# cloneofsimo/lora

Measured on AMD Instinct MI355X. Metric: train steps/sec SD1.5 rank-4 512^2 (train_lora_dreambooth.py step), higher is better.
Workload: dtype bf16

## Files before the change

include/lora_amd.h:

```cpp
#ifndef LORA_AMD_H
#define LORA_AMD_H

#include <stddef.h>
#include <stdint.h>

#ifdef __cplusplus
extern "C" {
#endif

#define LORA_AMD_ABI_VERSION 7

#define LORA_AMD_OK 0
#define LORA_AMD_EINVAL (-1)
#define LORA_AMD_ERANK (-2)
#define LORA_AMD_ELAUNCH (-3)
#define LORA_AMD_EWORKSPACE (-4)
#define LORA_AMD_EUNSUPPORTED (-5)

#define LORA_AMD_MAX_RANK 64

#define LORA_AMD_F32 0
#define LORA_AMD_F16 1
#define LORA_AMD_BF16 2

// ... 445 lines not shown
                                  int32_t r, int32_t act_dtype, float scale, float dropout_p, uint64_t seed, uint64_t offset,
                                  const uint64_t *offset_dev, void *stream);
int lora_amd_sum_parts(const float *part, int32_t nparts, int64_t stride, float *out, int64_t n, void *stream);


size_t lora_amd_sumsq_workspace(int64_t n);
int lora_amd_sumsq(const float *g, int64_t n, float *out_sumsq, void *workspace,
                   size_t workspace_bytes, void *stream);

typedef struct lora_amd_adamw_group {
  int64_t begin, end;
  float lr;
  float weight_decay;
} lora_amd_adamw_group;

int lora_amd_clip_adamw(float *p, float *g, float *exp_avg, float *exp_avg_sq,
                        int64_t n, const lora_amd_adamw_group *groups_dev,
                        int32_t n_groups, const float *sumsq, float grad_scale,
                        float max_norm, float beta1, float beta2, float eps,
                        int64_t step, int32_t zero_grad, void *stream);

int lora_amd_clip_adamw_dev(float *p, float *g, float *exp_avg, float *exp_avg_sq,
                            int64_t n, const lora_amd_adamw_group *groups_dev,
                            int32_t n_groups, const float *sumsq, float grad_scale,
                            float max_norm, float beta1, float beta2, float eps,
                            const int64_t *step_dev, const float *scaler, int32_t zero_grad, void *stream);
int lora_amd_step_advance(int64_t *step_dev, void *stream);

int lora_amd_loss_scale_update(float *state, const float *sumsq, int64_t *step_dev, float growth_factor,
                               float backoff_factor, int32_t growth_interval, void *stream);

int lora_amd_ti_rows_step(void *table, const void *table_grad, const int64_t *ids_dev, int32_t n_tokens,
                          int32_t hidden, int32_t table_dtype, float *rows, float *exp_avg, float *exp_avg_sq,
                          float lr, float beta1, float beta2, float eps, float weight_decay, float grad_scale,
                          int64_t step, float decay_lambda, float target_norm, void *stream);


size_t lora_amd_groupnorm_workspace(int32_t B, int32_t C, int32_t HW, int32_t groups);
int lora_amd_groupnorm_supported(int32_t B, int32_t C, int32_t HW, int32_t groups);
int lora_amd_groupnorm_fwd(const void *x, const void *gamma, const void *beta, void *y, float *stats,
                           void *workspace, size_t workspace_bytes, int32_t B, int32_t C, int32_t HW,
                           int32_t groups, float eps, int32_t act, int32_t dtype, void *stream);
int lora_amd_groupnorm_bwd(const void *x, const void *gout, const void *gamma, const void *beta,
                           const float *stats, void *dx, void *workspace, size_t workspace_bytes, int32_t B,
                           int32_t C, int32_t HW, int32_t groups, int32_t act, int32_t dtype, void *stream);

size_t lora_amd_groupnorm_nhwc_workspace(int32_t B, int32_t C, int32_t HW, int32_t groups);
int lora_amd_groupnorm_nhwc_fwd(const void *x, const void *gamma, const void *beta, const float *addend, void *y,
                                float *aff, void *workspace, size_t workspace_bytes, int32_t B, int32_t C, int32_t HW,
                                int32_t groups, float eps, int32_t act, int32_t dtype, void *stream);
int lora_amd_groupnorm_nhwc_bwd(const void *x, const void *gout, const void *gamma, const float *aff, void *dx,
                                void *workspace, size_t workspace_bytes, int32_t B, int32_t C, int32_t HW,
                                int32_t groups, int32_t act, int32_t dtype, void *stream);

int lora_amd_layernorm_supported(int32_t K);
int lora_amd_layernorm_fwd(const void *x, const void *gamma, const void *beta, void *y, float *stats, int64_t M,
                           int32_t K, float eps, int32_t dtype, void *stream);
int lora_amd_layernorm_bwd(const void *x, const void *gout, const void *gamma, const float *stats, void *dx,
                           int64_t M, int32_t K, int32_t dtype, void *stream);
int lora_amd_add_layernorm_fwd(const void *x, const void *res, const void *gamma, const void *beta, void *sum_out,
                               void *y, float *stats, int64_t M, int32_t K, float eps, int32_t dtype, void *stream);
int lora_amd_add_layernorm_bwd(const void *x, const void *gout, const void *gsum, const void *gamma,
                               const float *stats, void *dx, int64_t M, int32_t K, int32_t dtype, void *stream);

int lora_amd_geglu_fwd(const void *y, int64_t ldy, void *out, int64_t ldo, int64_t M, int32_t inner, int32_t dtype,
                       void *stream);
int lora_amd_geglu_bwd(const void *y, int64_t ldy, const void *gout, int64_t ldg, void *gy, int64_t ldgy, int64_t M,
                       int32_t inner, int32_t dtype, void *stream);

typedef struct lora_amd_attn_short_plan {
  int32_t run_blocks;
  int32_t slabs;
  int64_t slab_bytes;
  int64_t workspace_bytes;
} lora_amd_attn_short_plan;
int lora_amd_attn_short_bwd_supported(int64_t Sq, int32_t Sk, int32_t D, int32_t dtype, const int64_t *strides_host,
                                      int32_t n_strides);
int lora_amd_attn_short_bwd_plan(int32_t B, int32_t H, int64_t Sq, int32_t Sk, int32_t D,
                                 lora_amd_attn_short_plan *plan_host);
int lora_amd_attn_short_bwd(const void *q, const int64_t *q_strides_host, const void *k,
                            const int64_t *k_strides_host, const void *v, const int64_t *v_strides_host,
                            const void *dout, const int64_t *dout_strides_host, void *dq,
                            const int64_t *dq_strides_host, void *dk, const int64_t *dk_strides_host, void *dv,
                            const int64_t *dv_strides_host, int32_t B, int32_t H, int64_t Sq, int32_t Sk, int32_t D,
                            float scale, int32_t dtype, void *workspace, size_t workspace_bytes, void *stream);

#ifdef __cplusplus
}
#endif
#endif
```

lora_amd/_C.py:

```python
from __future__ import annotations

import ctypes as C
import os
from typing import Dict, Optional, Sequence, Tuple

import torch

_HERE = os.path.dirname(os.path.abspath(__file__))
LIB_PATH = os.path.join(_HERE, "csrc", "liblora_amd.so")

OK = 0
F32, F16, BF16 = 0, 1, 2
FACTOR_RK, FACTOR_KR = 0, 1
ROUND_REFERENCE, ROUND_ONCE, ROUND_DITHER = 0, 1, 2
MAX_RANK = 64
ABI_VERSION = 7

_DT = {torch.float32: F32, torch.float16: F16, torch.bfloat16: BF16}

class HipExtensionMissing(RuntimeError):
    pass


class AttnShortPlan(C.Structure):
# ... 292 lines not shown
    ("lora_amd_linear_ws_heads", cint, (vp, i64, i64, i32, i32, i32, i32, P(WsSite), i32, i32, vp)),
    ("lora_amd_linear_gemm_fwd_heads", cint, (vp, i64, vp, i64, vp, vp, i64, vp, vp, vp, i64, i32, i32, i32, i32,
        f32, f32, i32, i32, i32, i32, i32, i32, vp)),
    ("lora_amd_linear_gemm_fwd_rowscale", cint, (vp, i64, vp, i64, vp, vp, i64, vp, vp, vp, i64, i32, i32, i32, i32,
        f32, vp, i32, i64, i32, vp)),
    ("lora_amd_linear_factors_self_plan", cint, (i64, i32, i32, i32, P(FactorsSelfPlan))),
    ("lora_amd_linear_factors_self_plan_rows", cint, (i64, i32, i32, i32, i32, P(FactorsSelfPlan))),
    ("lora_amd_linear_bwd_factors_self", cint, (vp, i64, vp, i64, vp, vp, vp, vp, i64, i32, i32, i32, i32, f32, i32,
        i32, i32, i32, vp)),
    ("lora_amd_linear_factors_self_ragged_plan", cint, (vp, i32, i32, P(i64))),
    ("lora_amd_linear_bwd_factors_self_ragged", cint, (vp, i32, i64, i32, i32, vp)),
    ("lora_amd_reduce_batched", cint, (vp, i32, i64, vp)),
    ("lora_amd_factors_mfma_plan", cint, (i64, i32, i32, i32, i32, i32, i32, P(FactorsMfmaPlan))),
    ("lora_amd_factor_pack_plan", cint, (P(PackSite), i32, P(i64))),
    ("lora_amd_factor_pack", cint, (vp, i32, i64, i32, vp)),
    ("lora_amd_factors_mfma_ragged_plan", cint, (P(FmSite), i32, i32, i32, P(i64))),
    ("lora_amd_linear_bwd_factors_mfma_ragged", cint, (vp, i32, i64, i32, i32, i32, i32, vp)),
    ("lora_amd_factors_mfma_block_map", cint, (P(FmSite), i32, i64, P(i32))),
    ("lora_amd_linear_bwd_factors_mfma_ragged_mapped", cint, (vp, i32, i64, vp, i32, i32, i32, i32, vp)),
    ("lora_amd_factors_mfma_set_tuning", cint, (i32,)),
    ("lora_amd_conv_plan", cint, (i32, i32, i32, i32, i32, i32, i32, P(ConvPlan))),
    ("lora_amd_conv_down_fwd", cint, (vp, vp, vp, vp, vp, i32, i32, i32, i32, i32, i32, i32, i32, vp)),
    ("lora_amd_conv_up_fwd", cint, (vp, vp, vp, i32, i32, i32, i32, i32, i32, i32, f32, f32, u64, u64, vp, vp)),
    ("lora_amd_conv_up_fwd_rowscale", cint, (vp, vp, vp, i32, i32, i32, i32, i32, i32, i32, f32, vp, i32, i64, f32,
        u64, u64, vp)),
    ("lora_amd_conv_bwd_g", cint, (vp, vp, vp, vp, vp, vp, vp, i32, i32, i32, i32, i32, i32, i32, f32, f32, u64,
        u64, vp, vp)),
    ("lora_amd_conv_bwd_x", cint, (vp, vp, vp, vp, vp, i32, i32, i32, i32, i32, i32, i32, i32, vp)),
    ("lora_amd_conv3_nhwc_plan", cint, (i32, i32, i32, i32, i32, P(Conv3NhwcPlan))),
    ("lora_amd_conv3_nhwc_pack", cint, (vp, i32, i32, i32, vp, vp, vp)),
    ("lora_amd_conv3_nhwc_down_fwd", cint, (vp, vp, vp, vp, i32, i32, i32, i32, i32, i32, vp)),
    ("lora_amd_conv3_nhwc_bwd_dx", cint, (vp, vp, vp, i32, i32, i32, i32, i32, i32, vp)),
    ("lora_amd_conv3_nhwc_bwd_down", cint, (vp, vp, vp, i32, i32, i32, i32, i32, i32, vp)),
    ("lora_amd_conv3_nhwc_pack_plan", cint, (P(Conv3PackSite), i32, P(i64))),
    ("lora_amd_conv3_nhwc_pack_batched", cint, (vp, i32, i64, i32, vp)),
    ("lora_amd_conv3_nhwc_fwd_fused", cint, (vp, vp, vp, vp, vp, vp, vp, i32, i32, i32, i32, i32, i32, i32, f32,
        f32, u64, u64, vp, vp)),
    ("lora_amd_sum_parts", cint, (vp, i32, i64, vp, i64, vp)),
    ("lora_amd_sumsq_workspace", sz, (i64,)),
    ("lora_amd_sumsq", cint, (vp, i64, vp, vp, sz, vp)),
    ("lora_amd_clip_adamw", cint, (vp, vp, vp, vp, i64, vp, i32, vp, f32, f32, f32, f32, f32, i64, i32, vp)),
    ("lora_amd_clip_adamw_dev", cint, (vp, vp, vp, vp, i64, vp, i32, vp, f32, f32, f32, f32, f32, vp, vp, i32, vp)),
    ("lora_amd_step_advance", cint, (vp, vp)),
    ("lora_amd_loss_scale_update", cint, (vp, vp, vp, f32, f32, i32, vp)),
    ("lora_amd_ti_rows_step", cint, (vp, vp, vp, i32, i32, i32, vp, vp, vp, f32, f32, f32, f32, f32, f32, i64, f32,
        f32, vp)),
    ("lora_amd_groupnorm_workspace", sz, (i32, i32, i32, i32)),
    ("lora_amd_groupnorm_supported", cint, (i32, i32, i32, i32)),
    ("lora_amd_groupnorm_fwd", cint, (vp, vp, vp, vp, vp, vp, sz, i32, i32, i32, i32, f32, i32, i32, vp)),
    ("lora_amd_groupnorm_bwd", cint, (vp, vp, vp, vp, vp, vp, vp, sz, i32, i32, i32, i32, i32, i32, vp)),
    ("lora_amd_groupnorm_nhwc_workspace", sz, (i32, i32, i32, i32)),
    ("lora_amd_groupnorm_nhwc_fwd", cint, (vp, vp, vp, vp, vp, vp, vp, sz, i32, i32, i32, i32, f32, i32, i32, vp)),
    ("lora_amd_groupnorm_nhwc_bwd", cint, (vp, vp, vp, vp, vp, vp, sz, i32, i32, i32, i32, i32, i32, vp)),
    ("lora_amd_layernorm_supported", cint, (i32,)),
    ("lora_amd_layernorm_fwd", cint, (vp, vp, vp, vp, vp, i64, i32, f32, i32, vp)),
    ("lora_amd_layernorm_bwd", cint, (vp, vp, vp, vp, vp, i64, i32, i32, vp)),
    ("lora_amd_add_layernorm_fwd", cint, (vp, vp, vp, vp, vp, vp, vp, i64, i32, f32, i32, vp)),
    ("lora_amd_add_layernorm_bwd", cint, (vp, vp, vp, vp, vp, vp, i64, i32, i32, vp)),
    ("lora_amd_geglu_fwd", cint, (vp, i64, vp, i64, i64, i32, i32, vp)),
    ("lora_amd_geglu_bwd", cint, (vp, i64, vp, i64, vp, i64, i64, i32, i32, vp)),
    ("lora_amd_attn_short_bwd_supported", cint, (i64, i32, i32, i32, vp, i32)),
    ("lora_amd_attn_short_bwd_plan", cint, (i32, i32, i64, i32, i32, P(AttnShortPlan))),
    ("lora_amd_attn_short_bwd", cint, (vp, vp, vp, vp, vp, vp, vp, vp, vp, vp, vp, vp, vp, vp, i32, i32, i64, i32,
        i32, f32, i32, vp, sz, vp)),
)
SYMBOLS = tuple(name for name, _, _ in FUNCTIONS)


_lib: Optional[C.CDLL] = None
_load_error: Optional[str] = None


def _declare(lib: C.CDLL) -> None:
    for name, restype, argtypes in FUNCTIONS:
        fn = getattr(lib, name)
        fn.restype, fn.argtypes = restype, list(argtypes)


def load() -> Optional[C.CDLL]:
    global _lib, _load_error
    if _lib is not None or _load_error is not None:
        return _lib
    if not os.path.exists(LIB_PATH):
        _load_error = f"{LIB_PATH} not built (run `python -c 'import __graft_entry__ as g; g.build()'`)"
        return None
    try:
        lib = C.CDLL(LIB_PATH)
        _declare(lib)
        if lib.lora_amd_abi_version() != ABI_VERSION:
            raise OSError(f"ABI version {lib.lora_amd_abi_version()} != {ABI_VERSION} (rebuild: make -C lora_amd/csrc)")
        _lib = lib
    except OSError as e:
        _load_error = f"cannot load {LIB_PATH}: {e}"
    return _lib


def available() -> bool:
    return load() is not None


def require() -> C.CDLL:
    lib = load()
    if lib is None:
        raise HipExtensionMissing(
            "lora_amd: the HIP extension is required for device tensors and is not loadable: " + str(_load_error))
    return lib
# ... 1519 lines not shown
    elif out.dtype != y.dtype or tuple(out.shape) != shape or not out.is_contiguous():
        raise ValueError(f"geglu_fwd: out must be a contiguous {y.dtype} {list(shape)} tensor")
    _check(require().lora_amd_geglu_fwd(y2.data_ptr(), y2.stride(0), out.data_ptr(), inner, y2.shape[0], inner,
                                        dtype_code(y.dtype), _stream()), "lora_amd_geglu_fwd")
    return out


def geglu_bwd(y: torch.Tensor, gout: torch.Tensor) -> torch.Tensor:
    _dev_check(y, gout)
    y2, g2 = _as2d(y.reshape(-1, y.shape[-1])), _as2d(gout.reshape(-1, gout.shape[-1]))
    inner = y2.shape[1] // 2
    gy = torch.empty(y.shape, dtype=y.dtype, device=y.device)
    _check(require().lora_amd_geglu_bwd(y2.data_ptr(), y2.stride(0), g2.data_ptr(), g2.stride(0), gy.data_ptr(),
                                        2 * inner, y2.shape[0], inner, dtype_code(y.dtype), _stream()),
           "lora_amd_geglu_bwd")
    return gy


def layernorm_supported(K: int) -> bool:
    return bool(require().lora_amd_layernorm_supported(K))


def layernorm_fwd(x: torch.Tensor, gamma: torch.Tensor, beta: torch.Tensor, eps: float, *,
                  out: Optional[torch.Tensor] = None, stats: Optional[torch.Tensor] = None) -> Tuple[torch.Tensor, torch.Tensor]:
    _dev_check(x, gamma, beta, out, stats)
    K = x.shape[-1]
    M = x.numel() // K
    if out is None:
        y = torch.empty_like(x)
    elif out.dtype != x.dtype or out.shape != x.shape or not out.is_contiguous():
        raise ValueError("layernorm_fwd: out must be a contiguous tensor of x's shape and dtype")
    else:
        y = out
    if stats is None:
        stats = torch.empty(M, 2, dtype=torch.float32, device=x.device)
    elif stats.dtype != torch.float32 or tuple(stats.shape) != (M, 2) or not stats.is_contiguous():
        raise ValueError(f"layernorm_fwd: stats must be a contiguous f32 [{M}, 2] tensor")
    _check(require().lora_amd_layernorm_fwd(x.data_ptr(), gamma.data_ptr(), beta.data_ptr(), y.data_ptr(),
                                            stats.data_ptr(), M, K, eps, dtype_code(x.dtype), _stream()),
           "lora_amd_layernorm_fwd")
    return y, stats


def layernorm_bwd(x: torch.Tensor, gout: torch.Tensor, gamma: torch.Tensor, stats: torch.Tensor) -> torch.Tensor:
    _dev_check(x, gout, gamma, stats)
    K = x.shape[-1]
    dx = torch.empty_like(x)
    _check(require().lora_amd_layernorm_bwd(x.data_ptr(), gout.data_ptr(), gamma.data_ptr(), stats.data_ptr(),
                                            dx.data_ptr(), x.numel() // K, K, dtype_code(x.dtype), _stream()),
           "lora_amd_layernorm_bwd")
    return dx


_gn_nhwc_ws_cache: Dict[Tuple[int, int, int, int], int] = {}


def groupnorm_nhwc_workspace(B: int, C_: int, HW: int, groups: int) -> int:
    key = (B, C_, HW, groups)
    n = _gn_nhwc_ws_cache.get(key)
    if n is None:
        n = _gn_nhwc_ws_cache[key] = int(require().lora_amd_groupnorm_nhwc_workspace(B, C_, HW, groups))
    return n


def groupnorm_nhwc_fwd(x: torch.Tensor, gamma: torch.Tensor, beta: torch.Tensor, groups: int, eps: float,
                       act: bool, addend: Optional[torch.Tensor] = None) -> Tuple[torch.Tensor, torch.Tensor]:
    _dev_check(x, gamma, beta, addend)
    if addend is not None and (addend.dtype != torch.float32 or not addend.is_contiguous()
                               or tuple(addend.shape) != (x.shape[0], x.shape[1])):
        raise ValueError("groupnorm_nhwc_fwd: addend must be a contiguous float32 [B, C] tensor")
    B, C_ = x.shape[0], x.shape[1]
    HW = x.numel() // (B * C_)
    nbytes = groupnorm_nhwc_workspace(B, C_, HW, groups)
    if nbytes == 0:
        raise ValueError(f"lora_amd_groupnorm_nhwc: geometry {tuple(x.shape)} / {groups} groups not supported")
    y = torch.empty_like(x)
    aff = torch.empty(B, 4, C_, dtype=torch.float32, device=x.device)
    ws = torch.empty(nbytes // 4, dtype=torch.float32, device=x.device)
    _check(require().lora_amd_groupnorm_nhwc_fwd(x.data_ptr(), gamma.data_ptr(), beta.data_ptr(), _ptr(addend),
                                                 y.data_ptr(), aff.data_ptr(), ws.data_ptr(), nbytes, B, C_, HW, groups, eps,
                                                 1 if act else 0, dtype_code(x.dtype), _stream()),
           "lora_amd_groupnorm_nhwc_fwd")
    return y, aff


def groupnorm_nhwc_bwd(x: torch.Tensor, gout: torch.Tensor, gamma: torch.Tensor, aff: torch.Tensor, groups: int,
                       act: bool) -> torch.Tensor:
    _dev_check(x, gout, gamma, aff)
    B, C_ = x.shape[0], x.shape[1]
    HW = x.numel() // (B * C_)
    nbytes = groupnorm_nhwc_workspace(B, C_, HW, groups)
    dx = torch.empty_like(x)
    ws = torch.empty(nbytes // 4, dtype=torch.float32, device=x.device)
    _check(require().lora_amd_groupnorm_nhwc_bwd(x.data_ptr(), gout.data_ptr(), gamma.data_ptr(), aff.data_ptr(),
                                                 dx.data_ptr(), ws.data_ptr(), nbytes, B, C_, HW, groups,
                                                 1 if act else 0, dtype_code(x.dtype), _stream()),
           "lora_amd_groupnorm_nhwc_bwd")
    return dx


def add_layernorm_fwd(x: torch.Tensor, res: torch.Tensor, gamma: torch.Tensor, beta: torch.Tensor,
                      eps: float) -> Tuple[torch.Tensor, torch.Tensor, torch.Tensor]:
    _dev_check(x, res, gamma, beta)
    K = x.shape[-1]
    M = x.numel() // K
    s, y = torch.empty_like(x), torch.empty_like(x)
# ... 81 lines not shown
```

lora_amd/csrc/hostops.hip:

```cpp
#include <algorithm>

#include "common.hpp"

namespace lora_amd {

constexpr int kHT = 256;
constexpr int kHU = 4;
constexpr int kHMaxSlices = 256;

__device__ inline float fast_rcp(float v) { return __builtin_amdgcn_rcpf(v); }
__device__ inline float sigmoidf(float z) { return fast_rcp(1.f + __expf(-z)); }
__device__ inline float silu_grad(float z) {
  const float s = sigmoidf(z);
  return s * (1.f + z * (1.f - s));
}
__device__ inline float erf_as(float x) {
  const float ax = fabsf(x);
  const float t = fast_rcp(1.f + 0.3275911f * ax);
  float p = 1.061405429f;
  p = fmaf(p, t, -1.453152027f);
  p = fmaf(p, t, 1.421413741f);
  p = fmaf(p, t, -0.284496736f);
  p = fmaf(p, t, 0.254829592f);
  const float e = 1.f - p * t * __expf(-ax * ax);
// ... 752 lines not shown
      }
      LORA_AMD_LOADS_ISSUED();
#pragma unroll
      for (int u = 0; u < kNU; ++u) {
        const int pp = p + u * nslots;
        if (pp < k.np) {
          float v[8], go[8], t[8], xh[8];
          unpack8_sel<E>(xr[u], true, v);
          unpack8_sel<E>(gr[u], true, go);
          gn_nhwc_terms<E, ACT>(v, go, ga, be, mean, rstd, gam, t, xh);
          if (APPLY) {
            float o[8];
#pragma unroll
            for (int e = 0; e < 8; ++e) o[e] = rstd[e] * (t[e] - c1[e] - xh[e] * c2[e]);
            store8<E>(dx + k.base + (int64_t)pp * C, o);
          } else {
#pragma unroll
            for (int e = 0; e < 8; ++e) {
              s1[e] += t[e];
              s2[e] = fmaf(t[e], xh[e], s2[e]);
            }
          }
        }
      }
    }
  }
  if (!APPLY) {
    nhwc_slot_reduce(s1, s2, k, cw, nslots, s_red);
    if (k.active && k.slot == 0) {
      float *o = part + ((int64_t)(k.b * S + k.s) * 2) * C + (int64_t)k.col * 8;
      st8f(o, s1);
      st8f(o + C, s2);
    }
  }
}

__global__ __launch_bounds__(kHT) void gn_nhwc_bwd_finalize_kernel(const float *__restrict__ part,
                                                                   float *__restrict__ cvec, int C, int HW, int G,
                                                                   int S) {
  __shared__ float s_red[4][2];
  const int b = blockIdx.x / G, g = blockIdx.x - b * G, cpg = C / G;
  float s1 = 0.f, s2 = 0.f;
  for (int i = threadIdx.x; i < S * cpg; i += kHT) {
    const int s = i / cpg, c = g * cpg + (i - s * cpg);
    const float *pp = part + ((int64_t)(b * S + s) * 2) * C + c;
    s1 += pp[0];
    s2 += pp[C];
  }
  block_sum2(s1, s2, s_red);
  const float inv_n = 1.f / ((float)HW * (float)cpg);
  for (int cc = threadIdx.x; cc < cpg; cc += kHT) {
    cvec[(int64_t)b * 2 * C + g * cpg + cc] = s1 * inv_n;
    cvec[(int64_t)b * 2 * C + C + g * cpg + cc] = s2 * inv_n;
  }
}

static inline bool aligned_for(const void *p, int dt) { return ((uintptr_t)p % (dt == LORA_AMD_F32 ? 32 : 16)) == 0; }

}

using namespace lora_amd;

extern "C" size_t lora_amd_groupnorm_workspace(int32_t B, int32_t C, int32_t HW, int32_t groups) {
  const GnGeo q = gn_geo(B, C, HW, groups);
  return q.ok ? (size_t)B * groups * q.S * 2 * sizeof(float) : 0;
}

extern "C" int lora_amd_groupnorm_supported(int32_t B, int32_t C, int32_t HW, int32_t groups) {
  return gn_geo(B, C, HW, groups).ok ? 1 : 0;
}

#define GN_CHECKS(name)                                                                                              \
  const GnGeo q = gn_geo(B, C, HW, groups);                                                                          \
  LORA_AMD_CHECK(q.ok, LORA_AMD_EINVAL, name ": geometry B=%d C=%d HW=%d groups=%d not supported", B, C, HW, groups); \
  LORA_AMD_CHECK(dtype_ok(dtype), LORA_AMD_EINVAL, name ": bad dtype %d", dtype);                                    \
  LORA_AMD_CHECK(workspace_bytes >= lora_amd_groupnorm_workspace(B, C, HW, groups), LORA_AMD_EWORKSPACE,             \
                 name ": workspace %zu < %zu bytes", workspace_bytes, lora_amd_groupnorm_workspace(B, C, HW, groups)); \
  const dim3 grid((unsigned)((int64_t)B * groups * q.S)), block(kHT);                                                \
  hipStream_t st = (hipStream_t)stream;                                                                              \
  float *part = reinterpret_cast<float *>(workspace)

extern "C" int lora_amd_groupnorm_fwd(const void *x, const void *gamma, const void *beta, void *y, float *stats,
                                      void *workspace, size_t workspace_bytes, int32_t B, int32_t C, int32_t HW,
                                      int32_t groups, float eps, int32_t act, int32_t dtype, void *stream) {
  GN_CHECKS("groupnorm_fwd");
  LORA_AMD_CHECK(x && gamma && beta && y && stats && workspace, LORA_AMD_EINVAL, "groupnorm_fwd: null pointer");
  LORA_AMD_CHECK(aligned_for(x, dtype) && aligned_for(y, dtype), LORA_AMD_EINVAL, "groupnorm_fwd: unaligned tensor");
  by_dtype(dtype, [&](auto e) {
    using E = decltype(e);
    using S = typename E::storage;
    hipLaunchKernelGGL((gn_stats_kernel<E>), grid, block, 0, st, (const S *)x, part, groups, q.cpg, HW, q.chunks,
                       q.per_block, q.S);
    by_bool(act != 0, [&](auto a) {
      hipLaunchKernelGGL((gn_apply_kernel<E, decltype(a)::value>), grid, block, 0, st, (const S *)x, (const S *)gamma,
                         (const S *)beta, (S *)y, part, stats, groups, q.cpg, HW, q.chunks, q.per_block, q.S, eps);
    });
  });
  return check_launch("lora_amd_groupnorm_fwd");
}

extern "C" int lora_amd_groupnorm_bwd(const void *x, const void *gout, const void *gamma, const void *beta,
                                      const float *stats, void *dx, void *workspace, size_t workspace_bytes,
                                      int32_t B, int32_t C, int32_t HW, int32_t groups, int32_t act, int32_t dtype,
                                      void *stream) {
  GN_CHECKS("groupnorm_bwd");
  LORA_AMD_CHECK(x && gout && gamma && beta && stats && dx && workspace, LORA_AMD_EINVAL,
// ... 89 lines not shown
  const bool add = res != nullptr;
  by_dtype(dtype, [&](auto e) {
    by_bool(add, [&](auto a) {
      using S = typename decltype(e)::storage;
      hipLaunchKernelGGL((ln_fwd_kernel<decltype(e), decltype(a)::value>), grid, block, 0, st, (const S *)x, (const S *)res,
                         (const S *)gamma, (const S *)beta, (S *)sum_out, (S *)y, stats, M, c8, logL, eps);
    });
  });
  return check_launch("lora_amd_layernorm_fwd");
}

extern "C" int lora_amd_layernorm_bwd(const void *x, const void *gout, const void *gamma, const float *stats,
                                      void *dx, int64_t M, int32_t K, int32_t dtype, void *stream) {
  return lora_amd_add_layernorm_bwd(x, gout, nullptr, gamma, stats, dx, M, K, dtype, stream);
}

extern "C" int lora_amd_add_layernorm_bwd(const void *x, const void *gout, const void *gsum, const void *gamma,
                                          const float *stats, void *dx, int64_t M, int32_t K, int32_t dtype,
                                          void *stream) {
  LN_CHECKS("layernorm_bwd");
  LORA_AMD_CHECK(x && gout && gamma && stats && dx, LORA_AMD_EINVAL, "layernorm_bwd: null pointer");
  LORA_AMD_CHECK(aligned_for(x, dtype) && aligned_for(gout, dtype) && aligned_for(dx, dtype) && aligned_for(gamma, dtype) &&
                     aligned_for(gsum, dtype),
                 LORA_AMD_EINVAL, "layernorm_bwd: unaligned tensor");
  by_dtype(dtype, [&](auto e) {
    by_bool(gsum != nullptr, [&](auto a) {
      using S = typename decltype(e)::storage;
      hipLaunchKernelGGL((ln_bwd_kernel<decltype(e), decltype(a)::value>), grid, block, 0, st, (const S *)x, (const S *)gout,
                         (const S *)gsum, (const S *)gamma, stats, (S *)dx, M, c8, logL);
    });
  });
  return check_launch("lora_amd_layernorm_bwd");
}

static size_t gn_nhwc_part_floats(const GnNhwcGeo &q, int B, int C) { return (size_t)B * q.S * 2 * C; }

extern "C" size_t lora_amd_groupnorm_nhwc_workspace(int32_t B, int32_t C, int32_t HW, int32_t groups) {
  const GnNhwcGeo q = gn_nhwc_geo(B, C, HW, groups);
  return q.ok ? (gn_nhwc_part_floats(q, B, C) + (size_t)B * 2 * C) * sizeof(float) : 0;
}

#define GN_NHWC_CHECKS(name)                                                                                          \
  const GnNhwcGeo q = gn_nhwc_geo(B, C, HW, groups);                                                                  \
  LORA_AMD_CHECK(q.ok, LORA_AMD_EINVAL, name ": geometry B=%d C=%d HW=%d groups=%d not supported", B, C, HW, groups); \
  LORA_AMD_CHECK(dtype_ok(dtype), LORA_AMD_EINVAL, name ": bad dtype %d", dtype);                                     \
  LORA_AMD_CHECK(workspace_bytes >= lora_amd_groupnorm_nhwc_workspace(B, C, HW, groups), LORA_AMD_EWORKSPACE,         \
                 name ": workspace %zu bytes too small", workspace_bytes);                                            \
  const dim3 grid((unsigned)((int64_t)B * q.S * q.tiles)), gridg((unsigned)(B * groups)), block(kHT);                 \
  hipStream_t st = (hipStream_t)stream;                                                                               \
  float *part = reinterpret_cast<float *>(workspace);                                                                 \
  float *cvec = part + gn_nhwc_part_floats(q, B, C);                                                                  \
  (void)cvec

extern "C" int lora_amd_groupnorm_nhwc_fwd(const void *x, const void *gamma, const void *beta, const float *addend,
                                           void *y, float *aff, void *workspace, size_t workspace_bytes, int32_t B, int32_t C, int32_t HW,
                                           int32_t groups, float eps, int32_t act, int32_t dtype, void *stream) {
  GN_NHWC_CHECKS("groupnorm_nhwc_fwd");
  LORA_AMD_CHECK(x && gamma && beta && y && aff && workspace, LORA_AMD_EINVAL, "groupnorm_nhwc_fwd: null pointer");
  LORA_AMD_CHECK(aligned_for(x, dtype) && aligned_for(y, dtype) && ((uintptr_t)aff % 32) == 0, LORA_AMD_EINVAL,
                 "groupnorm_nhwc_fwd: unaligned tensor");
  by_dtype(dtype, [&](auto e) {
    using E = decltype(e);
    using S = typename E::storage;
    hipLaunchKernelGGL((gn_nhwc_stats_kernel<E>), grid, block, 0, st, (const S *)x, part, C, HW, q.cw, q.tiles,
                       q.nslots, q.px, q.S);
    hipLaunchKernelGGL((gn_nhwc_finalize_kernel<E>), gridg, block, 0, st, part, (const S *)gamma, (const S *)beta,
                       addend, aff, C, HW, groups, q.px, q.S, eps);
    by_bool(act != 0, [&](auto a) {
      hipLaunchKernelGGL((gn_nhwc_apply_kernel<E, decltype(a)::value>), grid, block, 0, st, (const S *)x, aff, (S *)y, C, HW,
                         q.cw, q.tiles, q.nslots, q.px, q.S);
    });
  });
  return check_launch("lora_amd_groupnorm_nhwc_fwd");
}

extern "C" int lora_amd_groupnorm_nhwc_bwd(const void *x, const void *gout, const void *gamma, const float *aff,
                                           void *dx, void *workspace, size_t workspace_bytes, int32_t B, int32_t C,
                                           int32_t HW, int32_t groups, int32_t act, int32_t dtype, void *stream) {
  GN_NHWC_CHECKS("groupnorm_nhwc_bwd");
  LORA_AMD_CHECK(x && gout && gamma && aff && dx && workspace, LORA_AMD_EINVAL, "groupnorm_nhwc_bwd: null pointer");
  LORA_AMD_CHECK(aligned_for(x, dtype) && aligned_for(gout, dtype) && aligned_for(dx, dtype) &&
                     aligned_for(gamma, dtype) && ((uintptr_t)aff % 32) == 0,
                 LORA_AMD_EINVAL, "groupnorm_nhwc_bwd: unaligned tensor");
  by_dtype(dtype, [&](auto e) {
    by_bool(act != 0, [&](auto a) {
      using E = decltype(e);
      using S = typename E::storage;
      constexpr bool A = decltype(a)::value;
      hipLaunchKernelGGL((gn_nhwc_bwd_kernel<E, A, false>), grid, block, 0, st, (const S *)x, (const S *)gout,
                         (const S *)gamma, aff, part, (const float *)nullptr, (S *)nullptr, C, HW, q.cw, q.tiles,
                         q.nslots, q.px, q.S);
      hipLaunchKernelGGL(gn_nhwc_bwd_finalize_kernel, gridg, block, 0, st, part, cvec, C, HW, groups, q.S);
      hipLaunchKernelGGL((gn_nhwc_bwd_kernel<E, A, true>), grid, block, 0, st, (const S *)x, (const S *)gout,
                         (const S *)gamma, aff, (float *)nullptr, cvec, (S *)dx, C, HW, q.cw, q.tiles, q.nslots,
                         q.px, q.S);
    });
  });
  return check_launch("lora_amd_groupnorm_nhwc_bwd");
}
```

lora_amd/ops.py:

```python
from __future__ import annotations

import os

from typing import NamedTuple, Optional

import torch
import torch.nn.functional as F

from . import _C

def next_dropout_stream(device) -> tuple:
    seed = int(torch.initial_seed()) & 0xFFFFFFFFFFFFFFFF
    pool = _POOL.get("buf")
    if pool is not None and pool.device == torch.device(device):
        i = _POOL["next"]
        if i >= pool.numel():
            pool = _POOL["buf"] = torch.empty(_POOL_SIZE, dtype=torch.int64, device=device).random_(0, 1 << 62)
            i = 0
        _POOL["next"] = i + 1
        return seed, pool[i:i + 1]
    off = torch.empty(1, dtype=torch.int64, device=device).random_(0, 1 << 62)
    return seed, off


# ... 385 lines not shown
            _log("bwd", "g+lib+x", M, K, N, r)
            gt_part, up_part, down_part = bufs()
            _C.linear_bwd_g(g2, t, up_c, gt_part, up_part, s, p, seed, off)
            dx2 = (g2 @ weight) if need_x else None
            if dx2 is not None and not _C._rows_ok(dx2):
                dx2 = dx2.contiguous()
            _C.linear_bwd_x(x2, dx2, gt_part, plan.nct_g, down_c, sel, down_part)
        if need_x:
            dx = dx2.view(x_shape)
        if not deferred:
            d_down, d_up = _finish(sink, site, bufs(), down, up)
    else:
        gt = None
        _log("bwd", "primitives", M, K, N, r)
        if need_x or need_down:
            gt = rowdot_any(g2, up_c, _C.FACTOR_KR, s, sel, True, p, seed, off)
        if need_up:
            if sink is not None:
                colreduce_any(g2, t, _C.FACTOR_KR, s, out=sink.up_grad, beta=1.0, p=p, seed=seed, off=off)
            else:
                d_up = colreduce_any(g2, t, _C.FACTOR_KR, s, p=p, seed=seed, off=off).to(up.dtype)
        if need_down:
            if sink is not None:
                colreduce_any(x2, gt, _C.FACTOR_RK, 1.0, out=sink.down_grad, beta=1.0)
            else:
                d_down = colreduce_any(x2, gt, _C.FACTOR_RK, 1.0).to(down.dtype)
        if need_x:
            dx2 = g2 @ weight
            rank_update_any_(dx2, gt, down_c, _C.FACTOR_RK, 1.0)
            dx = dx2.view(x_shape)
    dw = g2.t() @ x2 if need_w else None
    db = g2.sum(0) if (has_bias and need_b) else None
    return dx, dw, db, d_down, d_up


def _linear_backward_unpacked(ctx, g2, drop=(0.0, 0, 0)):
    x2, weight, down, up, t = ctx.saved_tensors[:5]
    x_log = unpack_heads(x2, ctx.in_heads) if ctx.in_heads else x2
    g_log = unpack_heads(g2, ctx.out_heads) if ctx.out_heads else g2
    dx, dw, db, d_down, d_up = _linear_backward(
        (x_log, weight, down, up, t, None), ctx.needs_input_grad[:5], g_log, ctx.scale, drop, ctx.sink,
        _C.fused_ok(x_log, weight.shape[0], down.shape[0]), ctx.has_bias, x_log.shape)
    if dx is not None:
        if ctx.in_heads:
            dx = pack_heads(dx, ctx.in_heads)
        dx = dx.view(*ctx.x_shape[:-1], dx.shape[-1])
    return dx, dw, db, d_down, d_up


CONCAT_GROUPS = True
CONV3_FUSED = True
MASTER_MERGE = True
ATTN_SHORT_BWD = True


def apply_ab_overrides(spec: str, namespace: dict) -> dict:
    allowed = ("ATTN_SHORT_BWD", "CONCAT_GROUPS", "CONV3_FUSED", "MASTER_MERGE", "WS_HEADS", "WS_DROPOUT", "WS_DROPOUT_WIDE",
               "WS_DROPOUT_WIDE_BWD")
    done = {}
    for item in filter(None, (s.strip() for s in spec.split(","))):
        name, _, val = item.partition("=")
        if name not in allowed:
            raise ValueError(f"LORA_AMD_AB: unknown constant {name!r} (one of {', '.join(allowed)})")
        namespace[name] = done[name] = val.strip() not in ("0", "", "false", "False")
    return done


apply_ab_overrides(os.environ.get("LORA_AMD_AB", ""), globals())

MERGE_ROUNDING = _C.ROUND_ONCE if os.environ.get("LORA_AMD_MERGE_ROUNDING", "dither") == "once" else _C.ROUND_DITHER


def master_site(w: torch.Tensor, dt: torch.dtype) -> bool:
    return MASTER_MERGE and w.dtype == torch.float32 and dt in (torch.bfloat16, torch.float16) and not w.requires_grad


def _gemm_range():
    if PATH_LOG is not None:
        return torch.profiler.record_function("lora_amd::merged_gemm")
    import contextlib

    return contextlib.nullcontext()


class MergedWeights:

    def __init__(self, state=None):
        self.entries = {}
        self._plans = None
        self.refreshes = 0
        self._state = state
        self._fresh_at = None
        self.defer_factors = state is not None
        self._owed = []
        self._tables = {}
        self._packs = {}
        self._pack_tables = {}
        self._graph_keep = []
        self.groups = {}
        self._keys = {}

    def lookup(self, module, w, b, dt, in_heads, out_heads, need_dx: bool = True):
        e = self._entry(module, w, b, dt, in_heads, out_heads)
        if need_dx and e["w_eff_t"] is None and (e["step"] or (in_heads is None and w.shape[0] % 32 == 0)):
            self._add_transposed(e)
        return e["w_eff"], e["b_eff"], e["w_eff_t"]

    def _refresh_if_stale(self) -> None:
        if (self._state is not None and self._fresh_at != self._state.step_count
                and not torch.cuda.is_current_stream_capturing()):
            self.refresh()

    def _entry(self, module, w, b, dt, in_heads, out_heads, out=None):
        self._refresh_if_stale()
        key = (id(module), in_heads, out_heads, dt)
        e = self.entries.get(key)
        if e is not None and (e["ptrs"] != (module.lora_up.weight.data_ptr(), module.lora_down.weight.data_ptr(),
                                            w.data_ptr()) or e["scale"] != float(module.scale)):
            if e.get("group") is not None:
                self.groups.pop(e["group"], None)
            e = None
# ... 1077 lines not shown
```

Baseline: 36.75.

## Add single-launch NHWC groupnorm forward/backward kernels for small spatial sizes

Adds one-kernel NHWC groupnorm forward and backward paths for HW up to 256. Each block keeps its pixel tile in registers and reduces group statistics in LDS with compensated sums, replacing the stats/finalize/apply sequence of three launches and the workspace round-trips. The path is on by default and can be switched off with an A/B override. In exchange, small-HW layers run with fewer blocks per launch and higher register pressure from the per-thread tiles.

New measurement: 36.97 (median of 4 runs). About the same (+0.6%).

```diff
diff --git a/include/lora_amd.h b/include/lora_amd.h
--- a/include/lora_amd.h
+++ b/include/lora_amd.h
@@ -521,6 +521,7 @@
 int lora_amd_groupnorm_nhwc_bwd(const void *x, const void *gout, const void *gamma, const float *aff, void *dx,
                                 void *workspace, size_t workspace_bytes, int32_t B, int32_t C, int32_t HW,
                                 int32_t groups, int32_t act, int32_t dtype, void *stream);
+int lora_amd_groupnorm_nhwc_set_tuning(int32_t one_launch);
 
 int lora_amd_layernorm_supported(int32_t K);
 int lora_amd_layernorm_fwd(const void *x, const void *gamma, const void *beta, void *y, float *stats, int64_t M,
diff --git a/lora_amd/_C.py b/lora_amd/_C.py
--- a/lora_amd/_C.py
+++ b/lora_amd/_C.py
@@ -368,6 +368,7 @@
     ("lora_amd_groupnorm_nhwc_workspace", sz, (i32, i32, i32, i32)),
     ("lora_amd_groupnorm_nhwc_fwd", cint, (vp, vp, vp, vp, vp, vp, vp, sz, i32, i32, i32, i32, f32, i32, i32, vp)),
     ("lora_amd_groupnorm_nhwc_bwd", cint, (vp, vp, vp, vp, vp, vp, sz, i32, i32, i32, i32, i32, i32, vp)),
+    ("lora_amd_groupnorm_nhwc_set_tuning", cint, (i32,)),
     ("lora_amd_layernorm_supported", cint, (i32,)),
     ("lora_amd_layernorm_fwd", cint, (vp, vp, vp, vp, vp, i64, i32, f32, i32, vp)),
     ("lora_amd_layernorm_bwd", cint, (vp, vp, vp, vp, vp, i64, i32, i32, vp)),
@@ -1993,6 +1994,10 @@
     return dx
 
 
+def groupnorm_nhwc_set_tuning(one_launch: int = -1) -> int:
+    return int(require().lora_amd_groupnorm_nhwc_set_tuning(int(one_launch)))
+
+
 _gn_nhwc_ws_cache: Dict[Tuple[int, int, int, int], int] = {}
 
 
diff --git a/lora_amd/csrc/hostops.hip b/lora_amd/csrc/hostops.hip
--- a/lora_amd/csrc/hostops.hip
+++ b/lora_amd/csrc/hostops.hip
@@ -828,6 +828,284 @@
   for (int cc = threadIdx.x; cc < cpg; cc += kHT) {
     cvec[(int64_t)b * 2 * C + g * cpg + cc] = s1 * inv_n;
     cvec[(int64_t)b * 2 * C + C + g * cpg + cc] = s2 * inv_n;
+  }
+}
+
+constexpr int kGnOneMaxHW = 256;
+constexpr int kGnOneMaxChunks = 32;
+
+struct GnOneGeo {
+  int cpg, nchunk, nblk, nslots, R;
+  bool ok;
+};
+static GnOneGeo gn_one_geo(int B, int C, int HW, int G, int dtype) {
+  GnOneGeo o{};
+  if (!(B > 0 && C > 0 && HW > 0 && G > 0 && C % G == 0 && C % 8 == 0)) return o;
+  o.cpg = C / G;
+  int cb = o.cpg;
+  while (cb % 8) cb += o.cpg;
+  o.nchunk = cb / 8;
+  o.nblk = C / cb;
+  if (HW > kGnOneMaxHW || o.nchunk > kGnOneMaxChunks) return o;
+  o.nslots = std::min(kHT / o.nchunk, HW);
+  o.R = (HW + o.nslots - 1) / o.nslots;
+  o.ok = o.R <= (dtype == LORA_AMD_F32 ? 8 : 16);
+  return o;
+}
+
+struct GnOneBlock {
+  int b, slot, cl, c;
+  bool active;
+  int64_t base;
+};
+__device__ inline GnOneBlock gn_one_block(int C, int HW, int nchunk, int nblk, int nslots) {
+  GnOneBlock k;
+  k.b = blockIdx.x / nblk;
+  const int blk = blockIdx.x - k.b * nblk;
+  k.slot = threadIdx.x / nchunk;
+  k.cl = (threadIdx.x - k.slot * nchunk) * 8;
+  k.active = k.slot < nslots;
+  k.c = blk * nchunk * 8 + k.cl;
+  k.base = (int64_t)k.b * HW * C + k.c;
+  return k;
+}
+
+struct GnOneLds {
+  float red[2 * kHT * 8];
+  float part[2][kHT];
+  float grp[2][kGnOneMaxChunks * 8];
+  float sh[kGnOneMaxChunks * 8];
+  float ad[kGnOneMaxChunks * 8];
+};
+
+__device__ inline void two_add(float &hi, float &lo, float v) {
+  const float t = hi + v, bb = t - hi;
+  lo += (hi - (t - bb)) + (v - bb);
+  hi = t;
+}
+__device__ inline void wave_two_sum(float &hi, float &lo) {
+#pragma unroll
+  for (int off = 32; off > 0; off >>= 1) {
+    const float oh = __shfl_xor(hi, off, 64), ol = __shfl_xor(lo, off, 64);
+    two_add(hi, lo, oh);
+    lo += ol;
+  }
+  const float t = hi + lo;
+  lo = (hi - t) + lo;
+  hi = t;
+}
+
+template <bool MEAN>
+__device__ inline void gn_one_group_avg(float (&a0)[8], float (&a1)[8], const GnOneBlock &k, int nchunk, int nslots, int cpg,
+                                        float denom, float inv_hw, GnOneLds &s) {
+  const int cb = nchunk * 8;
+  const int P = max(1, min(kHT / cb, nslots));
+  __syncthreads();
+  if (k.active) {
+    st8f(s.red + (size_t)threadIdx.x * 8, a0);
+    if (!MEAN) st8f(s.red + (size_t)(kHT + threadIdx.x) * 8, a1);
+  }
+  __syncthreads();
+  if ((int)threadIdx.x < P * cb) {
+    const int cls = threadIdx.x / cb, j = threadIdx.x - cls * cb;
+    float v0 = 0.f, v1 = 0.f;
+#pragma unroll 4
+    for (int sl = cls; sl < nslots; sl += P) {
+      v0 += s.red[sl * cb + j];
+      if (!MEAN) v1 += s.red[kHT * 8 + sl * cb + j];
+    }
+    s.part[0][threadIdx.x] = v0;
+    if (!MEAN) s.part[1][threadIdx.x] = v1;
+  }
+  __syncthreads();
+  const int wave = threadIdx.x >> 6, lane = threadIdx.x & 63;
+  for (int g = wave; g < cb / cpg; g += kHT / 64) {
+    float h0 = 0.f, l0 = 0.f, h1 = 0.f, l1 = 0.f;
+    for (int i = lane; i < P * cpg; i += 64) {
+      const int cls = i / cpg, j = g * cpg + (i - cls * cpg);
+      if (MEAN) {
+        two_add(h0, l0, s.part[0][cls * cb + j] * inv_hw);
+        if (cls == 0) {
+          two_add(h0, l0, s.sh[j]);
+          two_add(h0, l0, s.ad[j]);
+        }
+      } else {
+        two_add(h0, l0, s.part[0][cls * cb + j]);
+        two_add(h1, l1, s.part[1][cls * cb + j]);
+      }
+    }
+    wave_two_sum(h0, l0);
+    if (!MEAN) wave_two_sum(h1, l1);
+    if (lane == 0) {
+      const float q = h0 / denom;
+      s.grp[0][g] = q;
+      s.grp[1][g] = MEAN ? (fmaf(-q, denom, h0) + l0) / denom : h1 / denom;
+    }
+  }
+  __syncthreads();
+#pragma unroll
+  for (int e = 0; e < 8; ++e) {
+    const int g = (k.cl + e) / cpg;
+    a0[e] = s.grp[0][g];
+    a1[e] = s.grp[1][g];
+  }
+}
+
+template <class E, bool ACT, int R>
+__global__ __launch_bounds__(kHT) void gn_nhwc_one_fwd_kernel(const typename E::storage *__restrict__ x,
+                                                              const typename E::storage *__restrict__ gamma,
+                                                              const typename E::storage *__restrict__ beta,
+                                                              const float *__restrict__ addend,
+                                                              typename E::storage *__restrict__ y,
+                                                              float *__restrict__ aff, int C, int HW, int cpg, int nchunk,
+                                                              int nblk, int nslots, float eps) {
+  __shared__ __attribute__((aligned(16))) GnOneLds s;
+  const GnOneBlock k = gn_one_block(C, HW, nchunk, nblk, nslots);
+  Raw8<E> raw[R];
+#pragma unroll
+  for (int u = 0; u < R; ++u) {
+    const int pp = k.slot + u * nslots;
+    raw[u] = load8_raw<E>(x + k.base + (int64_t)(k.active && pp < HW ? pp : 0) * C);
+  }
+  const Raw8<E> shr = load8_raw<E>(x + k.base);
+  const Raw8<E> gr = load8_raw<E>(gamma + k.c), br = load8_raw<E>(beta + k.c);
+  float add[8];
+#pragma unroll
+  for (int e = 0; e < 8; ++e) add[e] = 0.f;
+  if (addend != nullptr) ld8f(addend + (int64_t)k.b * C + k.c, add);
+  LORA_AMD_LOADS_ISSUED();
+  float sh[8], a0[8], a1[8];
+  unpack8_sel<E>(shr, true, sh);
+#pragma unroll
+  for (int e = 0; e < 8; ++e) a0[e] = a1[e] = 0.f;
+#pragma unroll
+  for (int u = 0; u < R; ++u) {
+    float v[8];
+    unpack8_sel<E>(raw[u], true, v);
+    if (k.active && k.slot + u * nslots < HW) {
+#pragma unroll
+      for (int e = 0; e < 8; ++e) a0[e] += v[e] - sh[e];
+    }
+  }
+  if (k.slot == 0) {
+#pragma unroll
+    for (int e = 0; e < 8; ++e) {
+      s.sh[k.cl + e] = sh[e];
+      s.ad[k.cl + e] = add[e];
+    }
+  }
+  gn_one_group_avg<true>(a0, a1, k, nchunk, nslots, cpg, (float)cpg, 1.f / (float)HW, s);
+  float mc[8], ml[8];
+#pragma unroll
+  for (int e = 0; e < 8; ++e) {
+    float hi = a0[e], lo = a1[e];
+    two_add(hi, lo, -add[e]);
+    mc[e] = hi + lo;
+    ml[e] = (hi - mc[e]) + lo;
+    a0[e] = a1[e] = 0.f;
+  }
+#pragma unroll
+  for (int u = 0; u < R; ++u) {
+    float v[8];
+    unpack8_sel<E>(raw[u], true, v);
+    if (k.active && k.slot + u * nslots < HW) {
+#pragma unroll
+      for (int e = 0; e < 8; ++e) {
+        const float d = (v[e] - mc[e]) - ml[e];
+        a0[e] = fmaf(d, d, a0[e]);
+      }
+    }
+  }
+  gn_one_group_avg<false>(a0, a1, k, nchunk, nslots, cpg, (float)HW * (float)cpg, 0.f, s);
+  float gam[8], bet[8], ga[8], be[8], rstd[8];
+  unpack8_sel<E>(gr, true, gam);
+  unpack8_sel<E>(br, true, bet);
+#pragma unroll
+  for (int e = 0; e < 8; ++e) {
+    rstd[e] = rsqrtf(a0[e] + eps);
+    ga[e] = gam[e] * rstd[e];
+    be[e] = fmaf(-mc[e], ga[e], fmaf(-ml[e], ga[e], bet[e]));
+  }
+  if (!k.active) return;
+  if (k.slot == 0) {
+    float *o = aff + (int64_t)k.b * 4 * C + k.c;
+    st8f(o, ga);
+    st8f(o + C, be);
+    st8f(o + 2 * C, mc);
+    st8f(o + 3 * C, rstd);
+  }
+#pragma unroll
+  for (int u = 0; u < R; ++u) {
+    const int pp = k.slot + u * nslots;
+    if (pp < HW) {
+      float v[8], o[8];
+      unpack8_sel<E>(raw[u], true, v);
+#pragma unroll
+      for (int e = 0; e < 8; ++e) {
+        const float z = fmaf((v[e] - mc[e]) - ml[e], ga[e], bet[e]);
+        o[e] = ACT ? z * sigmoidf(z) : z;
+      }
+      store8<E>(y + k.base + (int64_t)pp * C, o);
+    }
+  }
+}
+
+template <class E, bool ACT, int R>
+__global__ __launch_bounds__(kHT) void gn_nhwc_one_bwd_kernel(const typename E::storage *__restrict__ x,
+                                                              const typename E::storage *__restrict__ gout,
+                                                              const typename E::storage *__restrict__ gamma,
+                                                              const float *__restrict__ aff,
+                                                              typename E::storage *__restrict__ dx, int C, int HW, int cpg,
+                                                              int nchunk, int nblk, int nslots) {
+  __shared__ __attribute__((aligned(16))) GnOneLds s;
+  const GnOneBlock k = gn_one_block(C, HW, nchunk, nblk, nslots);
+  Raw8<E> xr[R], gr[R];
+#pragma unroll
+  for (int u = 0; u < R; ++u) {
+    const int pp = k.slot + u * nslots;
+    const int64_t off = k.base + (int64_t)(k.active && pp < HW ? pp : 0) * C;
+    xr[u] = load8_raw<E>(x + off);
+    gr[u] = load8_raw<E>(gout + off);
+  }
+  float ga[8], be[8], mean[8], rstd[8], gam[8], s1[8], s2[8];
+  const float *ab = aff + (int64_t)k.b * 4 * C + k.c;
+  ld8f(ab, ga);
+  ld8f(ab + C, be);
+  ld8f(ab + 2 * C, mean);
+  ld8f(ab + 3 * C, rstd);
+  const Raw8<E> gmr = load8_raw<E>(gamma + k.c);
+  LORA_AMD_LOADS_ISSUED();
+  unpack8_sel<E>(gmr, true, gam);
+#pragma unroll
+  for (int e = 0; e < 8; ++e) s1[e] = s2[e] = 0.f;
+#pragma unroll
+  for (int u = 0; u < R; ++u) {
+    float v[8], go[8], t[8], xh[8];
+    unpack8_sel<E>(xr[u], true, v);
+    unpack8_sel<E>(gr[u], true, go);
+    gn_nhwc_terms<E, ACT>(v, go, ga, be, mean, rstd, gam, t, xh);
+    if (k.active && k.slot + u * nslots < HW) {
+#pragma unroll
+      for (int e = 0; e < 8; ++e) {
+        s1[e] += t[e];
+        s2[e] = fmaf(t[e], xh[e], s2[e]);
+      }
+    }
+  }
+  gn_one_group_avg<false>(s1, s2, k, nchunk, nslots, cpg, (float)HW * (float)cpg, 0.f, s);
+  if (!k.active) return;
+#pragma unroll
+  for (int u = 0; u < R; ++u) {
+    const int pp = k.slot + u * nslots;
+    if (pp < HW) {
+      float v[8], go[8], t[8], xh[8], o[8];
+      unpack8_sel<E>(xr[u], true, v);
+      unpack8_sel<E>(gr[u], true, go);
+      gn_nhwc_terms<E, ACT>(v, go, ga, be, mean, rstd, gam, t, xh);
+#pragma unroll
+      for (int e = 0; e < 8; ++e) o[e] = rstd[e] * (t[e] - s1[e] - xh[e] * s2[e]);
+      store8<E>(dx + k.base + (int64_t)pp * C, o);
+    }
   }
 }
 
@@ -1023,6 +1301,28 @@
   float *cvec = part + gn_nhwc_part_floats(q, B, C);                                                                  \
   (void)cvec
 
+static int g_gn_one_launch = 1;
+static unsigned g_gn_one_count = 0;
+
+extern "C" int lora_amd_groupnorm_nhwc_set_tuning(int32_t one_launch) {
+  if (one_launch == -2) return (int)(g_gn_one_count & 0x7fffffffu);
+  const int prev = g_gn_one_launch;
+  if (one_launch == 0 || one_launch == 1) g_gn_one_launch = one_launch;
+  return prev;
+}
+
+template <class E, class F>
+static void gn_one_by_tile(int R, F &&f) {
+  if (R <= 2) return f(int_c<2>);
+  if (R <= 4) return f(int_c<4>);
+  if constexpr (std::is_same<E, f32_t>::value) {
+    return f(int_c<8>);
+  } else {
+    if (R <= 8) return f(int_c<8>);
+    return f(int_c<16>);
+  }
+}
+
 extern "C" int lora_amd_groupnorm_nhwc_fwd(const void *x, const void *gamma, const void *beta, const float *addend,
                                            void *y, float *aff, void *workspace, size_t workspace_bytes, int32_t B, int32_t C, int32_t HW,
                                            int32_t groups, float eps, int32_t act, int32_t dtype, void *stream) {
@@ -1030,9 +1330,23 @@
   LORA_AMD_CHECK(x && gamma && beta && y && aff && workspace, LORA_AMD_EINVAL, "groupnorm_nhwc_fwd: null pointer");
   LORA_AMD_CHECK(aligned_for(x, dtype) && aligned_for(y, dtype) && ((uintptr_t)aff % 32) == 0, LORA_AMD_EINVAL,
                  "groupnorm_nhwc_fwd: unaligned tensor");
+  const GnOneGeo o = gn_one_geo(B, C, HW, groups, dtype);
+  const bool one = g_gn_one_launch != 0 && o.ok && aligned_for(gamma, dtype) && aligned_for(beta, dtype) &&
+                   ((uintptr_t)addend % 16) == 0;
   by_dtype(dtype, [&](auto e) {
     using E = decltype(e);
     using S = typename E::storage;
+    if (one) {
+      ++g_gn_one_count;
+      by_bool(act != 0, [&](auto a) {
+        gn_one_by_tile<E>(o.R, [&](auto rt) {
+          hipLaunchKernelGGL((gn_nhwc_one_fwd_kernel<E, decltype(a)::value, decltype(rt)::value>),
+                             dim3((unsigned)(B * o.nblk)), block, 0, st, (const S *)x, (const S *)gamma, (const S *)beta,
+                             addend, (S *)y, aff, C, HW, o.cpg, o.nchunk, o.nblk, o.nslots, eps);
+        });
+      });
+      return;
+    }
     hipLaunchKernelGGL((gn_nhwc_stats_kernel<E>), grid, block, 0, st, (const S *)x, part, C, HW, q.cw, q.tiles,
                        q.nslots, q.px, q.S);
     hipLaunchKernelGGL((gn_nhwc_finalize_kernel<E>), gridg, block, 0, st, part, (const S *)gamma, (const S *)beta,
@@ -1053,11 +1367,22 @@
   LORA_AMD_CHECK(aligned_for(x, dtype) && aligned_for(gout, dtype) && aligned_for(dx, dtype) &&
                      aligned_for(gamma, dtype) && ((uintptr_t)aff % 32) == 0,
                  LORA_AMD_EINVAL, "groupnorm_nhwc_bwd: unaligned tensor");
+  const GnOneGeo o = gn_one_geo(B, C, HW, groups, dtype);
+  const bool one = g_gn_one_launch != 0 && o.ok;
   by_dtype(dtype, [&](auto e) {
     by_bool(act != 0, [&](auto a) {
       using E = decltype(e);
       using S = typename E::storage;
       constexpr bool A = decltype(a)::value;
+      if (one) {
+        ++g_gn_one_count;
+        gn_one_by_tile<E>(o.R, [&](auto rt) {
+          hipLaunchKernelGGL((gn_nhwc_one_bwd_kernel<E, A, decltype(rt)::value>), dim3((unsigned)(B * o.nblk)), block, 0, st,
+                             (const S *)x, (const S *)gout, (const S *)gamma, aff, (S *)dx, C, HW, o.cpg, o.nchunk, o.nblk,
+                             o.nslots);
+        });
+        return;
+      }
       hipLaunchKernelGGL((gn_nhwc_bwd_kernel<E, A, false>), grid, block, 0, st, (const S *)x, (const S *)gout,
                          (const S *)gamma, aff, part, (const float *)nullptr, (S *)nullptr, C, HW, q.cw, q.tiles,
                          q.nslots, q.px, q.S);
diff --git a/lora_amd/ops.py b/lora_amd/ops.py
--- a/lora_amd/ops.py
+++ b/lora_amd/ops.py
@@ -461,11 +461,12 @@
 CONV3_FUSED = True
 MASTER_MERGE = True
 ATTN_SHORT_BWD = True
+GN_ONE_LAUNCH = True
 
 
 def apply_ab_overrides(spec: str, namespace: dict) -> dict:
-    allowed = ("ATTN_SHORT_BWD", "CONCAT_GROUPS", "CONV3_FUSED", "MASTER_MERGE", "WS_HEADS", "WS_DROPOUT", "WS_DROPOUT_WIDE",
-               "WS_DROPOUT_WIDE_BWD")
+    allowed = ("ATTN_SHORT_BWD", "CONCAT_GROUPS", "CONV3_FUSED", "GN_ONE_LAUNCH", "MASTER_MERGE", "WS_HEADS", "WS_DROPOUT",
+               "WS_DROPOUT_WIDE", "WS_DROPOUT_WIDE_BWD")
     done = {}
     for item in filter(None, (s.strip() for s in spec.split(","))):
         name, _, val = item.partition("=")
@@ -475,7 +476,8 @@
     return done
 
 
-apply_ab_overrides(os.environ.get("LORA_AMD_AB", ""), globals())
+if "GN_ONE_LAUNCH" in apply_ab_overrides(os.environ.get("LORA_AMD_AB", ""), globals()):
+    _C.groupnorm_nhwc_set_tuning(int(GN_ONE_LAUNCH))
 
 MERGE_ROUNDING = _C.ROUND_ONCE if os.environ.get("LORA_AMD_MERGE_ROUNDING", "dither") == "once" else _C.ROUND_DITHER
 
```
